# fani-lab/OpeNTF

Hardware: AMD Instinct MI355X
Metric: teams/sec (train) bnn_emb d=128 on DBLP (higher is better)
Workload: dtype f32 (fp16x3 split products, f32 accumulate)

## Files before the change

### opentf_amd/csrc/ntf_special.h

```cpp
#pragma once
#include "ntf_fused_common.h"

namespace ntf {

struct SpecialArgs {
    int B, M, Bpad, NCG, nCB, ns;
    int nslab;
    const float *h, *hs, *mu, *mu_b, *wp, *bp, *slab, *lossp, *h_mask;
    const uint32_t *sbits, *sinbits;
    const int64_t *rows, *m_indptr, *neg; const int32_t* m_indices;
    float tpw, tnw, inv_B;
    float *dzT, *dh, *row_fix;
    uint32_t so_k0, so_k1; int so_inj;
    float dz_pack_scale;
    const int* rflag;
    int c_lo;
    const uint16_t* wp_pl; float wp_inv_scale;
    int fb_ncg;
};

__device__ __forceinline__ int special_candidate(const int32_t* __restrict__ m_indices, const int64_t* __restrict__ neg, int64_t pb, int npos, int ns, int i, int sidx, float& y) {
    y = 0.f;
    if (sidx < npos) { y = 1.f; return m_indices[pb + sidx]; }
    const int qn = sidx - npos;
    if (!neg || qn >= ns) return -1;
    int c = (int)neg[(int64_t)i * ns + qn];
    for (int k = 0; k < npos; ++k) if (m_indices[pb + k] == c) c = -1;
    for (int k = 0; k < qn; ++k) if (c >= 0 && (int)neg[(int64_t)i * ns + k] == c) c = -1;
    return c;
}
template <bool BAYES>
__device__ __forceinline__ float special_z16(const float* __restrict__ mu, const float* __restrict__ mu_b, const float* __restrict__ wp, const float* __restrict__ bp,
                                             const uint16_t* __restrict__ wp_pl, float wp_inv_scale, bool wp_planes, const uint32_t* __restrict__ sbits, int nCB,
                                             uint32_t so_k0, uint32_t so_k1, int so_inj, int i, int cc, int l, const float (&hr)[8], const float (&hsr)[8],
                                             float (&mu_r)[8], float (&wp_r)[8], float& so) {
    constexpr int H = 128;
    float d1 = 0.f, d2 = 0.f;
    {
        const float4 a = *reinterpret_cast<const float4*>(mu + (int64_t)cc * H + 8 * l), b = *reinterpret_cast<const float4*>(mu + (int64_t)cc * H + 8 * l + 4);
        mu_r[0] = a.x; mu_r[1] = a.y; mu_r[2] = a.z; mu_r[3] = a.w; mu_r[4] = b.x; mu_r[5] = b.y; mu_r[6] = b.z; mu_r[7] = b.w;
    }
#pragma unroll
    for (int k = 0; k < 8; ++k) { d1 = fmaf(hr[k], mu_r[k], d1); wp_r[k] = 0.f; }
    if (BAYES) {
        if (wp_planes) {
            typedef _Float16 h8_t __attribute__((ext_vector_type(8)));
            const uint16_t* r0 = wp_pl + ((int64_t)(cc >> 5) * 64 + (cc & 31)) * H + 8 * l;
            const h8_t hi = *reinterpret_cast<const h8_t*>(r0), lo = *reinterpret_cast<const h8_t*>(r0 + 32 * H);
#pragma unroll
            for (int k = 0; k < 8; ++k) wp_r[k] = ((float)hi[k] + (float)lo[k]) * wp_inv_scale;
        } else {
            const float4 a = *reinterpret_cast<const float4*>(wp + (int64_t)cc * H + 8 * l), b = *reinterpret_cast<const float4*>(wp + (int64_t)cc * H + 8 * l + 4);
            wp_r[0] = a.x; wp_r[1] = a.y; wp_r[2] = a.z; wp_r[3] = a.w; wp_r[4] = b.x; wp_r[5] = b.y; wp_r[6] = b.z; wp_r[7] = b.w;
        }
#pragma unroll
        for (int k = 0; k < 8; ++k) d2 = fmaf(hsr[k], wp_r[k], d2);
    }
#pragma unroll
    for (int o = 8; o > 0; o >>= 1) d1 += __shfl_xor(d1, o, 64);
    float z = d1 + mu_b[cc];
    so = 1.f;
    if (BAYES) {
#pragma unroll
        for (int o = 8; o > 0; o >>= 1) d2 += __shfl_xor(d2, o, 64);
        const uint32_t sw_ = so_inj ? sbits[(int64_t)i * nCB + (cc >> 5)] : sign_word(so_k0, so_k1, (uint32_t)i, (uint32_t)(cc >> 5));
        so = ((sw_ >> (cc & 31)) & 1u) ? -1.f : 1.f;
        z += (d2 + bp[cc]) * so;
    }
    return z;
}
__device__ __forceinline__ float special_dz(float z, float y, float tpw, float inv_B, float& sp, float& sg, float& dact) {
    bce_terms(z, sp, sg, dact);
    return tpw * (sg - y) * dact * inv_B;
}
__device__ __forceinline__ uint32_t special_dz_packed(float dzt, float scale) { uint32_t pq[2]; split_pair_scaled(dzt, 0.f, scale, pq); return (pq[0] & 0xFFFFu) | (pq[1] << 16); }

void launch_out_special(hipStream_t st, int H, bool bayes, bool train, bool dh, const SpecialArgs& s);

}
```

### opentf_amd/csrc/ntf_special.hip

```cpp
#include "ntf_special.h"

namespace ntf {

template <int H, bool BAYES, bool TRAIN, bool DH>
__global__ __launch_bounds__(64) void k_out_special(SpecialArgs p) {
    constexpr bool QUAD = (H == 128);
    constexpr int NQ = QUAD ? 4 : 1;
    constexpr int NV = QUAD ? 8 : (H + 63) / 64;
    const int i = blockIdx.x, lane = threadIdx.x;
    const int q = QUAD ? (lane >> 4) : 0, l = QUAD ? (lane & 15) : lane;
    auto hidx = [&](int k) { return QUAD ? 8 * l + k : l + 64 * k; };
    const bool packed = p.dz_pack_scale > 0.f && !(p.rflag && *p.rflag);
    const bool wp_planes = BAYES && QUAD && p.wp_pl != nullptr && !(p.rflag && *p.rflag);
    const int ncg = (p.fb_ncg > 0 && p.rflag && *p.rflag) ? p.fb_ncg : p.NCG, nslab = (p.fb_ncg > 0 && p.rflag && *p.rflag) ? p.fb_ncg : p.nslab;
    float rl = 0.f;
    for (int cg = lane; cg < ncg; cg += 64) rl += p.lossp[(int64_t)i * ncg + cg];
    rl = wave_reduce_sum(rl);
    float acc[NV], hr[NV], hsr[NV];
#pragma unroll
    for (int k = 0; k < NV; ++k) {
        const int j = hidx(k);
        acc[k] = 0.f; hr[k] = 0.f; hsr[k] = 0.f;
        if (j < H) { hr[k] = p.h[(int64_t)i * H + j]; if (BAYES) hsr[k] = p.hs[(int64_t)i * H + j]; }
    }
    if (TRAIN && DH) {
        for (int cg = q; cg < nslab; cg += NQ) {
            const float* sl = p.slab + ((int64_t)cg * p.Bpad + i) * H;
#pragma unroll
            for (int k = 0; k < NV; ++k) { const int j = hidx(k); if (j < H) acc[k] += sl[j]; }
        }
    }
    auto group_sum = [&](float v) {
        if (!QUAD) return wave_reduce_sum(v);
#pragma unroll
        for (int o = 8; o > 0; o >>= 1) v += __shfl_xor(v, o, 64);
        return v;
    };
    const int64_t team = p.rows[i];
    const int64_t pb = p.m_indptr[team];
    const int npos = (int)(p.m_indptr[team + 1] - pb);
    const int total = npos + (p.neg ? p.ns : 0);
    float fix = 0.f;
    for (int s0 = 0; s0 < total; s0 += NQ) {
        const int sidx = s0 + q;
        float y = 0.f;
        int c = sidx < total ? special_candidate(p.m_indices, p.neg, pb, npos, p.ns, i, sidx, y) : -1;
        if (c >= 0) c -= p.c_lo;
        const bool live = c >= 0 && c < p.M;
        const int cc = live ? c : 0;
        float mu_r[NV], wp_r[NV], z, so = 1.f;
        if constexpr (QUAD) z = special_z16<BAYES>(p.mu, p.mu_b, p.wp, p.bp, p.wp_pl, p.wp_inv_scale, wp_planes, p.sbits, p.nCB, p.so_k0, p.so_k1, p.so_inj, i, cc, l, hr, hsr, mu_r, wp_r, so);
        else {
            float d1 = 0.f, d2 = 0.f;
#pragma unroll
            for (int k = 0; k < NV; ++k) {
                const int j = hidx(k);
                mu_r[k] = 0.f; wp_r[k] = 0.f;
                if (j < H) { mu_r[k] = p.mu[(int64_t)cc * H + j]; d1 += hr[k] * mu_r[k]; if (BAYES) { wp_r[k] = p.wp[(int64_t)cc * H + j]; d2 += hsr[k] * wp_r[k]; } }
            }
            d1 = group_sum(d1);
            z = d1 + p.mu_b[cc];
            if (BAYES) {
                d2 = group_sum(d2);
                const uint32_t sw_ = p.so_inj ? p.sbits[(int64_t)i * p.nCB + (cc >> 5)] : sign_word(p.so_k0, p.so_k1, (uint32_t)i, (uint32_t)(cc >> 5));
                so = ((sw_ >> (cc & 31)) & 1u) ? -1.f : 1.f;
                z += (d2 + p.bp[cc]) * so;
            }
        }
        float sp, sg, dact;
        const float dzt = special_dz(z, y, p.tpw, p.inv_B, sp, sg, dact);
        const float lz = z > 0.f ? z : z * kLeakySlope;
        if (live && l == 0) fix += p.tpw * (sp - lz * y) - p.tnw * sp;
        if (TRAIN && live) {
            const float delta = dzt - p.tnw * sg * dact * p.inv_B;
            if (l == 0) {
                if (packed) reinterpret_cast<uint32_t*>(p.dzT)[dzt_index(c, i, p.Bpad)] = special_dz_packed(dzt, p.dz_pack_scale);
                else p.dzT[dzt_index(c, i, p.Bpad)] = dzt;
            }
            if (DH) {
#pragma unroll
                for (int k = 0; k < NV; ++k) {
                    const int j = hidx(k);
                    if (j < H) {
                        acc[k] += delta * mu_r[k];
                        if (BAYES) {
                            const float si = ((p.sinbits[(int64_t)i * (H / 32) + (j >> 5)] >> (j & 31)) & 1u) ? -1.f : 1.f;
                            acc[k] += delta * so * wp_r[k] * si;
                        }
                    }
                }
            }
        }
    }
    if (QUAD) {
        fix += __shfl_xor(fix, 16, 64); fix += __shfl_xor(fix, 32, 64);
#pragma unroll
        for (int k = 0; k < NV; ++k) { acc[k] += __shfl_xor(acc[k], 16, 64); acc[k] += __shfl_xor(acc[k], 32, 64); }
    }
    if (lane == 0) p.row_fix[i] = rl + fix;
    if (TRAIN && DH && q == 0) {
#pragma unroll
        for (int k = 0; k < NV; ++k) {
            const int j = hidx(k);
            if (j < H) {
                float v = acc[k];
                if (p.h_mask) v *= (p.h_mask[(int64_t)i * H + j] > 0.f) ? 1.f : kLeakySlope;
                p.dh[(int64_t)i * H + j] = v;
            }
        }
    }
}

void launch_out_special(hipStream_t st, int H, bool bayes, bool train, bool dh, const SpecialArgs& s) {
#define NTF_SPK(HH, BY) do { if (!train) hipLaunchKernelGGL((k_out_special<HH, BY, false, false>), dim3(s.B), dim3(64), 0, st, s);         \
        else if (dh) hipLaunchKernelGGL((k_out_special<HH, BY, true, true>), dim3(s.B), dim3(64), 0, st, s);                                  \
        else hipLaunchKernelGGL((k_out_special<HH, BY, true, false>), dim3(s.B), dim3(64), 0, st, s); } while (0)
#define NTF_SPH(HH) do { if (bayes) NTF_SPK(HH, true); else NTF_SPK(HH, false); } while (0)
    if (H == 256) NTF_SPH(256); else if (H == 128) NTF_SPH(128); else if (H == 64) NTF_SPH(64); else NTF_SPH(32);
#undef NTF_SPH
#undef NTF_SPK
}

}
```

Measured before the change: 690,100.

## Prefetch candidate rows and slabs in special output kernel with register-held candidates

Restructures the per-team special output kernel so that candidate indices sit in wave registers and are deduplicated via readlane instead of repeated global scans. The mu/wp/bias/sign rows for upcoming candidates are fetched two steps ahead in a software pipeline. Slab partial sums are loaded in batches of eight, and loss partials, h_mask and sinbits are loaded up front so their latency overlaps other work. This hides global memory latency in a latency-bound one-wave-per-row kernel, at the cost of much higher register pressure, which may reduce occupancy.

```diff
diff --git a/opentf_amd/csrc/ntf_special.h b/opentf_amd/csrc/ntf_special.h
--- a/opentf_amd/csrc/ntf_special.h
+++ b/opentf_amd/csrc/ntf_special.h
@@ -29,43 +29,75 @@
     for (int k = 0; k < qn; ++k) if (c >= 0 && (int)neg[(int64_t)i * ns + k] == c) c = -1;
     return c;
 }
+__device__ __forceinline__ int special_candidate_held(int raw, int npos, int total, int sidx, float& y) {
+    y = (sidx < npos) ? 1.f : 0.f;
+    int c = __shfl(raw, sidx & 63, 64);
+    for (int k = 0; k < total; ++k) {
+        const int v = __builtin_amdgcn_readlane(raw, k);
+        if (sidx >= npos && k < sidx && v == c) c = -1;
+    }
+    return sidx < total ? c : -1;
+}
+template <int NV> struct SpecialRows { float mu_r[NV]; uint32_t w[NV]; float mb, bv; uint32_t sw; };
+typedef SpecialRows<8> SpecialRows16;
 template <bool BAYES>
-__device__ __forceinline__ float special_z16(const float* __restrict__ mu, const float* __restrict__ mu_b, const float* __restrict__ wp, const float* __restrict__ bp,
-                                             const uint16_t* __restrict__ wp_pl, float wp_inv_scale, bool wp_planes, const uint32_t* __restrict__ sbits, int nCB,
-                                             uint32_t so_k0, uint32_t so_k1, int so_inj, int i, int cc, int l, const float (&hr)[8], const float (&hsr)[8],
-                                             float (&mu_r)[8], float (&wp_r)[8], float& so) {
+__device__ __forceinline__ void special_rows16(const float* __restrict__ mu, const float* __restrict__ mu_b, const float* __restrict__ wp, const float* __restrict__ bp,
+                                               const uint16_t* __restrict__ wp_pl, bool wp_planes, const uint32_t* __restrict__ sbits, int nCB,
+                                               int so_inj, int i, int cc, int l, SpecialRows16& e) {
     constexpr int H = 128;
-    float d1 = 0.f, d2 = 0.f;
     {
         const float4 a = *reinterpret_cast<const float4*>(mu + (int64_t)cc * H + 8 * l), b = *reinterpret_cast<const float4*>(mu + (int64_t)cc * H + 8 * l + 4);
-        mu_r[0] = a.x; mu_r[1] = a.y; mu_r[2] = a.z; mu_r[3] = a.w; mu_r[4] = b.x; mu_r[5] = b.y; mu_r[6] = b.z; mu_r[7] = b.w;
+        e.mu_r[0] = a.x; e.mu_r[1] = a.y; e.mu_r[2] = a.z; e.mu_r[3] = a.w; e.mu_r[4] = b.x; e.mu_r[5] = b.y; e.mu_r[6] = b.z; e.mu_r[7] = b.w;
     }
+    e.mb = mu_b[cc]; e.bv = 0.f; e.sw = 0u;
 #pragma unroll
-    for (int k = 0; k < 8; ++k) { d1 = fmaf(hr[k], mu_r[k], d1); wp_r[k] = 0.f; }
+    for (int k = 0; k < 8; ++k) e.w[k] = 0u;
     if (BAYES) {
         if (wp_planes) {
             typedef _Float16 h8_t __attribute__((ext_vector_type(8)));
+            typedef uint32_t u4_t __attribute__((ext_vector_type(4)));
             const uint16_t* r0 = wp_pl + ((int64_t)(cc >> 5) * 64 + (cc & 31)) * H + 8 * l;
-            const h8_t hi = *reinterpret_cast<const h8_t*>(r0), lo = *reinterpret_cast<const h8_t*>(r0 + 32 * H);
+            const u4_t hi = __builtin_bit_cast(u4_t, *reinterpret_cast<const h8_t*>(r0)), lo = __builtin_bit_cast(u4_t, *reinterpret_cast<const h8_t*>(r0 + 32 * H));
 #pragma unroll
-            for (int k = 0; k < 8; ++k) wp_r[k] = ((float)hi[k] + (float)lo[k]) * wp_inv_scale;
+            for (int k = 0; k < 4; ++k) { e.w[k] = hi[k]; e.w[4 + k] = lo[k]; }
         } else {
             const float4 a = *reinterpret_cast<const float4*>(wp + (int64_t)cc * H + 8 * l), b = *reinterpret_cast<const float4*>(wp + (int64_t)cc * H + 8 * l + 4);
-            wp_r[0] = a.x; wp_r[1] = a.y; wp_r[2] = a.z; wp_r[3] = a.w; wp_r[4] = b.x; wp_r[5] = b.y; wp_r[6] = b.z; wp_r[7] = b.w;
+            e.w[0] = __float_as_uint(a.x); e.w[1] = __float_as_uint(a.y); e.w[2] = __float_as_uint(a.z); e.w[3] = __float_as_uint(a.w);
+            e.w[4] = __float_as_uint(b.x); e.w[5] = __float_as_uint(b.y); e.w[6] = __float_as_uint(b.z); e.w[7] = __float_as_uint(b.w);
+        }
+        e.bv = bp[cc];
+        if (so_inj) e.sw = sbits[(int64_t)i * nCB + (cc >> 5)];
+    }
+}
+template <bool BAYES>
+__device__ __forceinline__ float special_z16(const SpecialRows16& e, float wp_inv_scale, bool wp_planes, uint32_t so_k0, uint32_t so_k1, int so_inj, int i, int cc, const float (&hr)[8], const float (&hsr)[8], float (&wp_r)[8], float& so) {
+    float d1 = 0.f, d2 = 0.f;
+#pragma unroll
+    for (int k = 0; k < 8; ++k) { d1 = fmaf(hr[k], e.mu_r[k], d1); wp_r[k] = 0.f; }
+    if (BAYES) {
+        if (wp_planes) {
+#pragma unroll
+            for (int k = 0; k < 8; ++k) {
+                const uint16_t hb = (uint16_t)(e.w[k >> 1] >> (16 * (k & 1))), lb = (uint16_t)(e.w[4 + (k >> 1)] >> (16 * (k & 1)));
+                wp_r[k] = ((float)__builtin_bit_cast(_Float16, hb) + (float)__builtin_bit_cast(_Float16, lb)) * wp_inv_scale;
+            }
+        } else {
+#pragma unroll
+            for (int k = 0; k < 8; ++k) wp_r[k] = __uint_as_float(e.w[k]);
         }
 #pragma unroll
         for (int k = 0; k < 8; ++k) d2 = fmaf(hsr[k], wp_r[k], d2);
     }
 #pragma unroll
     for (int o = 8; o > 0; o >>= 1) d1 += __shfl_xor(d1, o, 64);
-    float z = d1 + mu_b[cc];
+    float z = d1 + e.mb;
     so = 1.f;
     if (BAYES) {
 #pragma unroll
         for (int o = 8; o > 0; o >>= 1) d2 += __shfl_xor(d2, o, 64);
-        const uint32_t sw_ = so_inj ? sbits[(int64_t)i * nCB + (cc >> 5)] : sign_word(so_k0, so_k1, (uint32_t)i, (uint32_t)(cc >> 5));
+        const uint32_t sw_ = so_inj ? e.sw : sign_word(so_k0, so_k1, (uint32_t)i, (uint32_t)(cc >> 5));
         so = ((sw_ >> (cc & 31)) & 1u) ? -1.f : 1.f;
-        z += (d2 + bp[cc]) * so;
+        z += (d2 + e.bv) * so;
     }
     return z;
 }
diff --git a/opentf_amd/csrc/ntf_special.hip b/opentf_amd/csrc/ntf_special.hip
--- a/opentf_amd/csrc/ntf_special.hip
+++ b/opentf_amd/csrc/ntf_special.hip
@@ -7,64 +7,113 @@
     constexpr bool QUAD = (H == 128);
     constexpr int NQ = QUAD ? 4 : 1;
     constexpr int NV = QUAD ? 8 : (H + 63) / 64;
+    constexpr int SLAB_B = 8;
     const int i = blockIdx.x, lane = threadIdx.x;
     const int q = QUAD ? (lane >> 4) : 0, l = QUAD ? (lane & 15) : lane;
     auto hidx = [&](int k) { return QUAD ? 8 * l + k : l + 64 * k; };
+    const int64_t team = p.rows[i];
     const bool packed = p.dz_pack_scale > 0.f && !(p.rflag && *p.rflag);
     const bool wp_planes = BAYES && QUAD && p.wp_pl != nullptr && !(p.rflag && *p.rflag);
     const int ncg = (p.fb_ncg > 0 && p.rflag && *p.rflag) ? p.fb_ncg : p.NCG, nslab = (p.fb_ncg > 0 && p.rflag && *p.rflag) ? p.fb_ncg : p.nslab;
-    float rl = 0.f;
-    for (int cg = lane; cg < ncg; cg += 64) rl += p.lossp[(int64_t)i * ncg + cg];
-    rl = wave_reduce_sum(rl);
-    float acc[NV], hr[NV], hsr[NV];
+    float acc[NV], hr[NV], hsr[NV], hm[NV];
+    uint32_t sinw[NV];
 #pragma unroll
     for (int k = 0; k < NV; ++k) {
         const int j = hidx(k);
-        acc[k] = 0.f; hr[k] = 0.f; hsr[k] = 0.f;
+        acc[k] = 0.f; hr[k] = 0.f; hsr[k] = 0.f; hm[k] = 1.f; sinw[k] = 0u;
         if (j < H) { hr[k] = p.h[(int64_t)i * H + j]; if (BAYES) hsr[k] = p.hs[(int64_t)i * H + j]; }
     }
-    if (TRAIN && DH) {
-        for (int cg = q; cg < nslab; cg += NQ) {
+    if (TRAIN && DH && p.h_mask) {
+#pragma unroll
+        for (int k = 0; k < NV; ++k) { const int j = hidx(k); if (j < H) hm[k] = p.h_mask[(int64_t)i * H + j]; }
+    }
+    if (TRAIN && DH && BAYES) {
+#pragma unroll
+        for (int k = 0; k < NV; ++k) { const int j = hidx(k); if (j < H) sinw[k] = p.sinbits[(int64_t)i * (H / 32) + (j >> 5)]; }
+    }
+    auto slab_load = [&](int cg0, float (&sv)[SLAB_B][NV]) {
+#pragma unroll
+        for (int u = 0; u < SLAB_B; ++u) {
+            const int cg = cg0 + u * NQ < nslab ? cg0 + u * NQ : nslab - 1;
             const float* sl = p.slab + ((int64_t)cg * p.Bpad + i) * H;
 #pragma unroll
-            for (int k = 0; k < NV; ++k) { const int j = hidx(k); if (j < H) acc[k] += sl[j]; }
-        }
-    }
+            for (int k = 0; k < NV; ++k) { const int j = hidx(k); sv[u][k] = j < H ? sl[j] : 0.f; }
+        }
+    };
+    auto slab_add = [&](int cg0, const float (&sv)[SLAB_B][NV]) {
+#pragma unroll
+        for (int u = 0; u < SLAB_B; ++u) {
+            const bool in = cg0 + u * NQ < nslab;
+#pragma unroll
+            for (int k = 0; k < NV; ++k) { const int j = hidx(k); if (j < H) acc[k] = in ? acc[k] + sv[u][k] : acc[k]; }
+        }
+    };
+    const bool slabs = TRAIN && DH && nslab > 0;
+    float sv0[SLAB_B][NV];
+#pragma unroll
+    for (int u = 0; u < SLAB_B; ++u)
+#pragma unroll
+        for (int k = 0; k < NV; ++k) sv0[u][k] = 0.f;
+    if (slabs) slab_load(q, sv0);
     auto group_sum = [&](float v) {
         if (!QUAD) return wave_reduce_sum(v);
 #pragma unroll
         for (int o = 8; o > 0; o >>= 1) v += __shfl_xor(v, o, 64);
         return v;
     };
-    const int64_t team = p.rows[i];
     const int64_t pb = p.m_indptr[team];
     const int npos = (int)(p.m_indptr[team + 1] - pb);
     const int total = npos + (p.neg ? p.ns : 0);
-    float fix = 0.f;
-    for (int s0 = 0; s0 < total; s0 += NQ) {
-        const int sidx = s0 + q;
-        float y = 0.f;
-        int c = sidx < total ? special_candidate(p.m_indices, p.neg, pb, npos, p.ns, i, sidx, y) : -1;
-        if (c >= 0) c -= p.c_lo;
-        const bool live = c >= 0 && c < p.M;
-        const int cc = live ? c : 0;
-        float mu_r[NV], wp_r[NV], z, so = 1.f;
-        if constexpr (QUAD) z = special_z16<BAYES>(p.mu, p.mu_b, p.wp, p.bp, p.wp_pl, p.wp_inv_scale, wp_planes, p.sbits, p.nCB, p.so_k0, p.so_k1, p.so_inj, i, cc, l, hr, hsr, mu_r, wp_r, so);
+    const bool held = total <= 64;
+    int raw = -1;
+    if (held && lane < total) raw = lane < npos ? p.m_indices[pb + lane] : (int)p.neg[(int64_t)i * p.ns + (lane - npos)];
+    const bool rl_first = lane < ncg;
+    float rl0 = 0.f;
+    if (rl_first) rl0 = p.lossp[(int64_t)i * ncg + lane];
+    struct Entry { int c, cc; float y; bool live; SpecialRows<NV> r; };
+    auto fetch = [&](int c, float y, Entry& e) {
+        e.c = c; e.y = y;
+        if (e.c >= 0) e.c -= p.c_lo;
+        e.live = e.c >= 0 && e.c < p.M;
+        e.cc = e.live ? e.c : 0;
+        if constexpr (QUAD) special_rows16<BAYES>(p.mu, p.mu_b, p.wp, p.bp, p.wp_pl, wp_planes, p.sbits, p.nCB, p.so_inj, i, e.cc, l, e.r);
+        else {
+#pragma unroll
+            for (int k = 0; k < NV; ++k) {
+                const int j = hidx(k);
+                e.r.mu_r[k] = 0.f; e.r.w[k] = 0u;
+                if (j < H) { e.r.mu_r[k] = p.mu[(int64_t)e.cc * H + j]; if (BAYES) e.r.w[k] = __float_as_uint(p.wp[(int64_t)e.cc * H + j]); }
+            }
+            e.r.mb = p.mu_b[e.cc]; e.r.bv = 0.f; e.r.sw = 0u;
+            if (BAYES) {
+                e.r.bv = p.bp[e.cc];
+                if (p.so_inj) e.r.sw = p.sbits[(int64_t)i * p.nCB + (e.cc >> 5)];
+            }
+        }
+    };
+    auto fetch_held = [&](int s0, Entry& e) { float y; const int c = special_candidate_held(raw, npos, total, s0 + q, y); fetch(c, y, e); };
+    float sik[NV], fix = 0.f;
+    auto reduce = [&](const Entry& e) {
+        const int c = e.c, cc = e.cc;
+        const bool live = e.live;
+        const float y = e.y;
+        float wp_r[NV], z, so = 1.f;
+        if constexpr (QUAD) z = special_z16<BAYES>(e.r, p.wp_inv_scale, wp_planes, p.so_k0, p.so_k1, p.so_inj, i, cc, hr, hsr, wp_r, so);
         else {
             float d1 = 0.f, d2 = 0.f;
 #pragma unroll
             for (int k = 0; k < NV; ++k) {
                 const int j = hidx(k);
-                mu_r[k] = 0.f; wp_r[k] = 0.f;
-                if (j < H) { mu_r[k] = p.mu[(int64_t)cc * H + j]; d1 += hr[k] * mu_r[k]; if (BAYES) { wp_r[k] = p.wp[(int64_t)cc * H + j]; d2 += hsr[k] * wp_r[k]; } }
+                wp_r[k] = 0.f;
+                if (j < H) { d1 += hr[k] * e.r.mu_r[k]; if (BAYES) { wp_r[k] = __uint_as_float(e.r.w[k]); d2 += hsr[k] * wp_r[k]; } }
             }
             d1 = group_sum(d1);
-            z = d1 + p.mu_b[cc];
+            z = d1 + e.r.mb;
             if (BAYES) {
                 d2 = group_sum(d2);
-                const uint32_t sw_ = p.so_inj ? p.sbits[(int64_t)i * p.nCB + (cc >> 5)] : sign_word(p.so_k0, p.so_k1, (uint32_t)i, (uint32_t)(cc >> 5));
+                const uint32_t sw_ = p.so_inj ? e.r.sw : sign_word(p.so_k0, p.so_k1, (uint32_t)i, (uint32_t)(cc >> 5));
                 so = ((sw_ >> (cc & 31)) & 1u) ? -1.f : 1.f;
-                z += (d2 + p.bp[cc]) * so;
+                z += (d2 + e.r.bv) * so;
             }
         }
         float sp, sg, dact;
@@ -82,15 +131,45 @@
                 for (int k = 0; k < NV; ++k) {
                     const int j = hidx(k);
                     if (j < H) {
-                        acc[k] += delta * mu_r[k];
+                        acc[k] += delta * e.r.mu_r[k];
                         if (BAYES) {
-                            const float si = ((p.sinbits[(int64_t)i * (H / 32) + (j >> 5)] >> (j & 31)) & 1u) ? -1.f : 1.f;
+                            const float si = sik[k];
                             acc[k] += delta * so * wp_r[k] * si;
                         }
                     }
                 }
             }
         }
+    };
+    Entry cur = {}, nxt = {}, nx2 = {};
+    if (held && total > 0) {
+        fetch_held(0, cur);
+        if (total > NQ) { fetch_held(NQ, nxt); if (total > 2 * NQ) fetch_held(2 * NQ, nx2); }
+    }
+    if (slabs) {
+        slab_add(q, sv0);
+        for (int cg0 = q + NQ * SLAB_B; cg0 < nslab; cg0 += NQ * SLAB_B) { float sv[SLAB_B][NV]; slab_load(cg0, sv); slab_add(cg0, sv); }
+    }
+    float rl = 0.f;
+    if (rl_first) rl += rl0;
+    for (int cg = lane + 64; cg < ncg; cg += 64) rl += p.lossp[(int64_t)i * ncg + cg];
+    rl = wave_reduce_sum(rl);
+#pragma unroll
+    for (int k = 0; k < NV; ++k) { const int j = hidx(k); sik[k] = ((sinw[k] >> (j & 31)) & 1u) ? -1.f : 1.f; }
+    if (held) {
+        for (int s0 = 0; s0 < total; s0 += NQ) {
+            reduce(cur);
+            cur = nxt; nxt = nx2;
+            if (s0 + 3 * NQ < total) fetch_held(s0 + 3 * NQ, nx2);
+        }
+    } else {
+        for (int s0 = 0; s0 < total; s0 += NQ) {
+            const int sidx = s0 + q;
+            float y = 0.f;
+            const int c = sidx < total ? special_candidate(p.m_indices, p.neg, pb, npos, p.ns, i, sidx, y) : -1;
+            fetch(c, y, cur);
+            reduce(cur);
+        }
     }
     if (QUAD) {
         fix += __shfl_xor(fix, 16, 64); fix += __shfl_xor(fix, 32, 64);
@@ -104,7 +183,7 @@
             const int j = hidx(k);
             if (j < H) {
                 float v = acc[k];
-                if (p.h_mask) v *= (p.h_mask[(int64_t)i * H + j] > 0.f) ? 1.f : kLeakySlope;
+                if (p.h_mask) v *= (hm[k] > 0.f) ? 1.f : kLeakySlope;
                 p.dh[(int64_t)i * H + j] = v;
             }
         }
```

New measurement: 687,000. No clear change (-0.4%).
